# xfause/OpenGL_Ray_Tracing

Hardware: AMD Instinct MI355X
Metric: Mrays/sec + ms/frame (1 spp, 1080p) at 1/2/4/8 MI355X; CPU-ref spp-matched PSNR (higher is better)
Workload: dtype f32; 1 GPU; c2: OpenglRayTracing bunny scene (5k tris), 1080p, 1 spp/frame, Lambert; resolution=1920x1080, spp_per_frame=1, integrator=lambert, max_bounce=2, triangles=5004, bvh_nodes=2826, bvh_builder=sah, env=peppermint, traversal_tree=runtime (checked against uploaded), frame_kernel=path regeneration, frames_in_flight=2, hw_queues=4, frames_per_launch=12, parallelism=screen-tile x1

## Files before the change

opengl_ray_tracing_amd/csrc/pt_device.h:

```cpp
#pragma once
#include <hip/hip_runtime.h>
#include <stdint.h>

#include "pt_fmath.h"
#include "pt_kernels.h"

#define PT_PI 3.1415926f
#define PT_INF 2147483647.0f

namespace pt {

struct V3 {
  float x, y, z;
};
__device__ __forceinline__ V3 v3(float x, float y, float z) { return V3{x, y, z}; }
__device__ __forceinline__ V3 operator+(V3 a, V3 b) { return v3(a.x + b.x, a.y + b.y, a.z + b.z); }
__device__ __forceinline__ V3 operator-(V3 a, V3 b) { return v3(a.x - b.x, a.y - b.y, a.z - b.z); }
__device__ __forceinline__ V3 operator*(V3 a, V3 b) { return v3(a.x * b.x, a.y * b.y, a.z * b.z); }
__device__ __forceinline__ V3 operator*(V3 a, float s) { return v3(a.x * s, a.y * s, a.z * s); }
__device__ __forceinline__ V3 operator/(V3 a, float s) { return v3(a.x / s, a.y / s, a.z / s); }
__device__ __forceinline__ V3 operator-(V3 a) { return v3(-a.x, -a.y, -a.z); }
__device__ __forceinline__ float dot(V3 a, V3 b) { return (a.x * b.x + a.y * b.y) + a.z * b.z; }
__device__ __forceinline__ V3 cross(V3 a, V3 b) {
  return v3(a.y * b.z - b.y * a.z, a.z * b.x - b.z * a.x, a.x * b.y - b.x * a.y);
// ... 206 lines not shown
  b = b + 0.5f;
  u = a;
  w = 1.0f - b;
}
__device__ __noinline__ int sphTexelExact(int W, int H, V3 v) {
  float u, w;
  toSpherical(v, u, w);
  return texIndex(W, H, u, w);
}
__device__ __forceinline__ int sphTexel(int W, int H, V3 v) {
  float a = ptm_atan2f_fast(v.z, v.x), b = ptm_asinf_fast(v.y);
  a = a / (2.0f * PT_PI);
  b = b / PT_PI;
  a = a + 0.5f;
  b = b + 0.5f;
  const float fx = a * (float)W, fy = (1.0f - b) * (float)H;
  if (fabsf(fx - rintf(fx)) > 4e-7f * (float)W && fabsf(fy - rintf(fy)) > 4e-7f * (float)H) {
    const int x = (int)fminf(fmaxf(floorf(fx), 0.0f), (float)(W - 1));
    const int y = (int)fminf(fmaxf(floorf(fy), 0.0f), (float)(H - 1));
    return y * W + x;
  }
  return sphTexelExact(W, H, v);
}
__device__ __forceinline__ V3 sampleHdr(const Env& e, V3 v) {
  if (!e.hdr) return v3(0, 0, 0);
  float4 c = envTexelK(e, sphTexel(e.w, e.h, normalize(v)));
  return v3(fminf(c.x, 10.0f), fminf(c.y, 10.0f), fminf(c.z, 10.0f));
}
__device__ __forceinline__ V3 hdrColor(const Env& e, V3 L) {
  if (!e.hdr) return v3(0, 0, 0);
  float u, w;
  toSpherical(normalize(L), u, w);
  float4 c = envTexel(e, u, w);
  return v3(c.x, c.y, c.z);
}
__device__ __forceinline__ float2 hdrCacheTexel(const Env& e, float xi1, float xi2) {
  if (!e.cache) return make_float2(0.0f, 0.0f);
  if (e.cacheRow) {
    int col, row;
    texXY(e.w, e.h, xi1, xi2, col, row);
    const uint32_t r = e.cacheRow[row];
    const uint32_t y = e.cacheY[(size_t)(r >> 16) * e.w + (col & ((PT_DIAG_ENV_SMALL & 2) ? 1023 : -1))];
    return decodeCache4((r & 0xffffu) | y << 16, e.w, e.h);
  }
  const int k = texIndex(e.w, e.h, xi1, xi2) & ((PT_DIAG_ENV_SMALL & 2) ? 1023 : -1);
  if (e.nt) return e.cache4 ? decodeCache4(ldStream(e.cache4 + k), e.w, e.h) : ldStream(e.cache + k);
  return e.cache4 ? decodeCache4(e.cache4[k], e.w, e.h) : e.cache[k];
}
__device__ __forceinline__ float hdrTheta(float y) { return PT_PI * ((1.0f - y) - 0.5f); }
__device__ __forceinline__ float hdrPhi(float x) { return 2.0f * PT_PI * (x - 0.5f); }
// ... 288 lines not shown
```

opengl_ray_tracing_amd/csrc/pt_display.hip:

```cpp
#include <hip/hip_runtime.h>

#include <stdint.h>

#include "pt_device.h"
#include "pt_frame.h"
#include "pt_kernels.h"

namespace pt {

__global__ void tonemapKernel(const float4* accum, float* rgb, int n, float limit, float gamma) {
  int i = blockIdx.x * blockDim.x + threadIdx.x;
  if (i >= n) return;
  const V3 c = tonemapPixel(accum[i], limit, gamma);
  rgb[3 * i] = c.x;
  rgb[3 * i + 1] = c.y;
  rgb[3 * i + 2] = c.z;
}
hipError_t launchTonemap(const float4* accum, float* rgb, int n, float limit, float gamma, hipStream_t s) {
  hipLaunchKernelGGL(tonemapKernel, dim3((n + 255) / 256), dim3(256), 0, s, accum, rgb, n, limit, gamma);
  return hipGetLastError();
}
__device__ __forceinline__ uint32_t unorm8(float x) {
  const float c = fminf(fmaxf(x, 0.0f), 1.0f);
  return (uint32_t)__builtin_fmaf(c, 255.0f, 0.5f);
// ... 138 lines not shown
  if (!src) return;
  PackParams p = d.base;
  p.share.rank = rank;
  p.count = d.count[rank];
  long k = (long)blockIdx.x * blockDim.x + threadIdx.x;
  if (k >= p.count) return;
  int px, py;
  if (!pixelOfSlot(p.share, k, px, py)) return;
  const float* in = src + PACK_STATS_F * k;
  const size_t i = (size_t)py * p.share.width + px;
  stStream(accum + i, make_float4(in[0], in[1], in[2], 1.0f));
  stStream(moments + i, make_float2(in[3], in[4]));
}
hipError_t launchUnpackRanksStats(const RanksUnpack& d, int world, float4* accum, float2* moments, hipStream_t s) {
  if (!accum || !moments) return hipErrorInvalidValue;
  long most = 0;
  for (int k = 1; k < world; k++) most = d.count[k] > most ? d.count[k] : most;
  if (world < 2 || most <= 0) return hipSuccess;
  hipLaunchKernelGGL(unpackRanksStatsKernel, dim3((unsigned)((most + 255) / 256), (unsigned)(world - 1)), dim3(256), 0,
                     s, d, accum, moments);
  return hipGetLastError();
}

template <bool MOMENTS, bool ADAPTIVE = false>
__device__ __forceinline__ void mixFrames(const PackParams& p, float4* accum, float2* moments, const float* col,
                                          size_t colStride, int nFrames, uint32_t frameCounter,
                                          const uint32_t* retiredAt = nullptr) {
  long k = (long)blockIdx.x * blockDim.x + threadIdx.x;
  if (k >= p.count) return;
  int px, py;
  if (!pixelOfSlot(p.share, k, px, py)) return;
  if (ADAPTIVE && retiredAt[(size_t)(py >> 3) * ((p.share.width + 7) >> 3) + (px >> 3)] != 0u) return;
  const size_t i = (size_t)py * p.share.width + px;
  float4 a = ldStream(accum + i);
  float2 m = make_float2(0.0f, 0.0f);
  if (MOMENTS) m = ldStream(moments + i);
  for (int f = 0; f < nFrames; f++) {
    const float3 c = ldCol(col + ((size_t)f * colStride + k) * COL_F);
    const float w = 1.0f / (float)(frameCounter + (uint32_t)f + 1u);
    a = make_float4(mixf(a.x, c.x, w), mixf(a.y, c.y, w), mixf(a.z, c.z, w), 1.0f);
    if (MOMENTS) {
      const float l = (0.3f * c.x + 0.6f * c.y) + 0.1f * c.z;
      m = make_float2(mixf(m.x, l, w), mixf(m.y, l * l, w));
    }
  }
  stStream(accum + i, a);
  if (MOMENTS) stStream(moments + i, m);
}
__global__ void mixKernel(PackParams p, float4* accum, const float* col, size_t colStride, int nFrames,
                          uint32_t frameCounter) {
  mixFrames<false>(p, accum, nullptr, col, colStride, nFrames, frameCounter);
}
__global__ void mixMomentsKernel(PackParams p, float4* accum, float2* moments, const float* col, size_t colStride,
                                 int nFrames, uint32_t frameCounter) {
  mixFrames<true>(p, accum, moments, col, colStride, nFrames, frameCounter);
}
__global__ void mixAdaptiveKernel(PackParams p, float4* accum, float2* moments, const float* col, size_t colStride,
                                  int nFrames, uint32_t frameCounter, const uint32_t* retiredAt) {
  mixFrames<true, true>(p, accum, moments, col, colStride, nFrames, frameCounter, retiredAt);
}
hipError_t launchMix(const PackParams& p, float4* accum, const float* col, size_t colStride, int nFrames,
                     uint32_t frameCounter, hipStream_t s) {
  if (p.count <= 0 || nFrames <= 0) return hipSuccess;
  hipLaunchKernelGGL(mixKernel, dim3((unsigned)((p.count + 255) / 256)), dim3(256), 0, s, p, accum, col, colStride,
                     nFrames, frameCounter);
  return hipGetLastError();
}
hipError_t launchMixMoments(const PackParams& p, float4* accum, float2* moments, const float* col, size_t colStride,
                            int nFrames, uint32_t frameCounter, hipStream_t s) {
  if (p.count <= 0 || nFrames <= 0) return hipSuccess;
  hipLaunchKernelGGL(mixMomentsKernel, dim3((unsigned)((p.count + 255) / 256)), dim3(256), 0, s, p, accum, moments, col,
                     colStride, nFrames, frameCounter);
  return hipGetLastError();
}
hipError_t launchMixAdaptive(const PackParams& p, float4* accum, float2* moments, const float* col, size_t colStride,
                             int nFrames, uint32_t frameCounter, const uint32_t* retiredAt, hipStream_t s) {
  if (!retiredAt) return hipErrorInvalidValue;
  if (p.count <= 0 || nFrames <= 0) return hipSuccess;
  hipLaunchKernelGGL(mixAdaptiveKernel, dim3((unsigned)((p.count + 255) / 256)), dim3(256), 0, s, p, accum, moments,
                     col, colStride, nFrames, frameCounter, retiredAt);
  return hipGetLastError();
}

}
```

opengl_ray_tracing_amd/csrc/pt_kernels.h:

```cpp
#pragma once
#include <hip/hip_runtime.h>
#include <stdint.h>

namespace pt {

#ifndef PT_BLOCK
#define PT_BLOCK 256
#endif
constexpr int BLOCK = PT_BLOCK;
#ifndef PT_LDS_STACK
#define PT_LDS_STACK 32
#endif
#ifndef PT_MIN_WAVES_LAMBERT
#define PT_MIN_WAVES_LAMBERT 3
#endif
#ifndef PT_COST_EMA
#define PT_COST_EMA 2
#endif
#ifndef PT_WIDE_SCENE_MB
#define PT_WIDE_SCENE_MB 48
#endif
constexpr int WIDE_WAVES = 3;
#ifndef PT_WIDE_REGEN_WAVES
#define PT_WIDE_REGEN_WAVES 4
// ... 234 lines not shown
  const void* src[DISPLAY_MAX_WORLD];
  long count[DISPLAY_MAX_WORLD];
};

#ifndef PT_BIN_CAP
#define PT_BIN_CAP 32
#endif
#ifndef PT_PASS_BIN_CAP
#define PT_PASS_BIN_CAP 64
#endif
#ifndef PT_BINS
#define PT_BINS 1
#endif
struct PrimaryBins {
  int4* rect = nullptr;
  int* triCount = nullptr;
  int* triOffset = nullptr;
  int* tileCount = nullptr;
  int* binStart = nullptr;
  int* binTris = nullptr;
  float4* binGeo = nullptr;
  float4* binBox = nullptr;
  void* tmp = nullptr;
  size_t rectCap = 0, triCountCap = 0, triOffsetCap = 0, tileCountCap = 0, binStartCap = 0, binTrisCap = 0,
         binGeoCap = 0, binBoxCap = 0, tmpBytes = 0;
  int tilesX = 0, tilesY = 0, entries = 0;
};
hipError_t buildPrimaryBins(const float eye[3], const float cam[16], int width, int height, const float4* geo,
                            const float4* leafBox, int nTri, PrimaryBins& b, hipStream_t s);
void freePrimaryBins(PrimaryBins& b);

struct BuildNode {
  float4 lo;
  float4 hi;
  float4 clo;
  float4 chi;
};
struct AccelBuild {
  float4* bvh = nullptr;
  float4* pairs = nullptr;
  int* order = nullptr;
  BuildNode* nodes = nullptr;
  int rootRef = REF_NONE, nDev = 0, depth = 0, nNodes = 0;
};
hipError_t buildAccelDevice(const float4* geo, int nTri, int leafSize, float inflate, float inflateRelAbs,
                            AccelBuild& out, hipStream_t s);
void freeAccelBuild(AccelBuild& a);
hipError_t collapseWide4Device(const BuildNode* nodes, int nNodes, int leafSize, float inflate, float inflateRelAbs,
                               float4** out, int* rootRef, int* nDev, int* depth, hipStream_t s);

struct RefitTables {
  int2* topo = nullptr;
// ... 34 lines not shown
  const float* mats;
  int stride;
  int nTri;
  float4* hitRec;
  float4* table;
};
int materialSlots(int nTri);
hipError_t materialScanBytes(int nTri, size_t* bytes);
hipError_t launchMaterials(const MaterialParams& p, const MaterialTables& t, hipEvent_t* ev, hipStream_t s);

hipError_t launchHdrCache(const float* hdr, int w, int h, float4* cache, float* scratch, hipStream_t s);
hipError_t launchEnvCompact(const float4* hdr, const float2* cache, int w, int h, uint2* hdr8, uint32_t* cache4,
                            int* bad, hipStream_t s);
hipError_t launchEnvPack(float4* hdr, const float4* cache, float2* samp, int n, hipStream_t s);
hipError_t launchEnvTrig(float2* trig, int w, int h, hipStream_t s);
hipError_t launchEnvLight(const Env& e, uint2* light, hipStream_t s);
hipError_t launchRender(const RenderParams& p, int integrator, int grid, hipStream_t s, bool cull, bool count,
                        bool wide = false);
constexpr int REORDER_MAX = 4096;
hipError_t launchReorder(int* cost, int* costMax, int* splitLg, int* ema, int* order, int perQueue, int orderCap,
                         int numItems, int group, int numWaves, int splitPct, hipStream_t s);
hipError_t renderBlocksPerCU(int integrator, bool cull, bool count, bool wide, int* nb);
constexpr int PRIM_MISS = -1, PRIM_RETRACE = -2, PRIM_TILE = -3;
hipError_t launchPrimary(const RenderParams& p, hipStream_t s);
hipError_t launchLiveList(const RenderParams& p, hipStream_t s);
struct RegenVariant {
  const void* fn = nullptr;
  int waves = 0;
  int block = BLOCK;
  bool lists = true;
  int top4 = 0;
};
struct RegenShape {
  bool wide = false;
  bool fullTree = false;
  bool small = false;
  RegenVariant v;
  int blocksPerCU = 0;
  size_t dynLds = 0;
};
hipError_t regenShape(int integrator, bool cull, bool wide, int f4nDev, bool smallScene, RegenShape* out);
hipError_t launchRegen(const RenderParams& p, int integrator, int grid, hipStream_t s, bool cull, const RegenShape& r);
bool regenTakesLists(int integrator, const RegenShape& r);
int regenLdsStack();
int regenTop4(const RegenShape& r, int integrator);
hipError_t launchQuery(const QueryParams& p, int grid, hipStream_t s, bool occluded, bool cull);
struct GuideParams {
// ... 65 lines not shown
  float sigmaZ, normalCos, maxHistory;
  float frames;
};
constexpr int TEMPORAL_TILE = 16;
hipError_t launchTemporal(const TemporalParams& p, hipStream_t s);
hipError_t launchBasic(const BasicParams& p, hipStream_t s);
hipError_t launchBasicWiden(const float4* accum, double* image, long n, hipStream_t s);
hipError_t launchBasicNarrow(const double* image, float4* accum, long n, hipStream_t s);
hipError_t launchTonemap(const float4* accum, float* rgb, int n, float limit, float gamma, hipStream_t s);
constexpr int PACK_F = 3;
hipError_t launchPack(const PackParams& p, const float4* accum, float* packed, hipStream_t s);
hipError_t launchFmath(int fn, const float* x, const float* y, int n, float* out, hipStream_t s);
hipError_t launchSphTexel(int W, int H, const float* dirs, int n, int* texel, int* texelExact, hipStream_t s);
hipError_t launchDisplayPack(const PackParams& p, const float4* accum, float limit, float gamma, uint8_t* packed,
                             hipStream_t s);
hipError_t launchDisplayOwn(const PackParams& p, const float4* accum, float limit, float gamma, uchar4* image,
                            hipStream_t s);
hipError_t launchDisplayUnpack(const RanksUnpack& d, int world, uchar4* image, hipStream_t s);
hipError_t launchUnpackRanks(const RanksUnpack& d, int world, float4* accum, hipStream_t s);
hipError_t launchUnpack(const PackParams& p, float4* accum, const float* packed, hipStream_t s);
constexpr int PACK_STATS_F = 5;
hipError_t launchPackStats(const PackParams& p, const float4* accum, const float2* moments, float* packed, hipStream_t s);
hipError_t launchUnpackRanksStats(const RanksUnpack& d, int world, float4* accum, float2* moments, hipStream_t s);
hipError_t launchMix(const PackParams& p, float4* accum, const float* col, size_t colStride, int nFrames,
                     uint32_t frameCounter, hipStream_t s);
hipError_t launchMixMoments(const PackParams& p, float4* accum, float2* moments, const float* col, size_t colStride,
                            int nFrames, uint32_t frameCounter, hipStream_t s);
hipError_t launchMixAdaptive(const PackParams& p, float4* accum, float2* moments, const float* col, size_t colStride,
                             int nFrames, uint32_t frameCounter, const uint32_t* retiredAt, hipStream_t s);
struct TileErrorParams {
  Share share;
  int shardTiles;
  int waveTiles;
  int tilesX;
  const float4* accum;
  const float2* moments;
  float* err2;
  uint32_t* retiredAt;
  float kf;
  float limit;
  float thr2;
  uint32_t frames;
  int minFrames;
};
hipError_t launchTileError(const TileErrorParams& p, hipStream_t s);

}
```

opengl_ray_tracing_amd/csrc/pt_primary.hip:

```cpp
#include <hip/hip_runtime.h>
#include <hipcub/hipcub.hpp>
#include <stdint.h>

#include "pt_frame.h"
#include "pt_kernels.h"
#include "pt_trace.h"

namespace pt {

struct BinCam {
  double eye[3];
  double R[9];
  int width, height, tilesX, tilesY;
};

constexpr double kNearZ = -2.5e-4;
constexpr double kMarginPx = 2.0;

__device__ __forceinline__ void toCam(const BinCam& c, const float4 v, double q[3]) {
  const double r0 = (double)v.x - c.eye[0], r1 = (double)v.y - c.eye[1], r2 = (double)v.z - c.eye[2];
  for (int a = 0; a < 3; a++) q[a] = c.R[3 * a] * r0 + c.R[3 * a + 1] * r1 + c.R[3 * a + 2] * r2;
}

__global__ void binRectKernel(BinCam c, const float4* geo, int nTri, int4* rect, int* count) {
// ... 135 lines not shown
  if ((e = hipMemcpyAsync(&entries, b.triOffset + nTri, sizeof(int), hipMemcpyDeviceToHost, s)) != hipSuccess) return e;
  if ((e = hipStreamSynchronize(s)) != hipSuccess) return e;
  if ((e = grow(b.binTris, b.binTrisCap, (size_t)std::max(entries, 1))) != hipSuccess) return e;
  if ((e = hipMemsetAsync(b.tileCount, 0, ((size_t)nTiles + 1) * sizeof(int), s)) != hipSuccess) return e;
  if (entries > 0)
    hipLaunchKernelGGL(binCountKernel, dim3((entries + B - 1) / B), dim3(B), 0, s, b.triOffset, b.rect, nTri, c.tilesX,
                       entries, b.tileCount);
  if ((e = scanInts(b.tileCount, b.binStart, nTiles, b.tmp, b.tmpBytes, s)) != hipSuccess) return e;
  if ((e = hipMemsetAsync(b.tileCount, 0, ((size_t)nTiles + 1) * sizeof(int), s)) != hipSuccess) return e;
  if (entries > 0)
    hipLaunchKernelGGL(binFillKernel, dim3((entries + B - 1) / B), dim3(B), 0, s, b.triOffset, b.rect, nTri, c.tilesX,
                       entries, b.binStart, b.tileCount, b.binTris);
  if ((e = grow(b.binGeo, b.binGeoCap, 4 * (size_t)std::max(entries, 1))) != hipSuccess) return e;
  if ((e = grow(b.binBox, b.binBoxCap, 2 * (size_t)std::max(entries, 1))) != hipSuccess) return e;
  if (entries > 0 && leafBox)
    hipLaunchKernelGGL(binGatherKernel, dim3((entries + B - 1) / B), dim3(B), 0, s, b.binTris, entries, geo, leafBox,
                       b.binGeo, b.binBox);
  b.tilesX = c.tilesX;
  b.tilesY = c.tilesY;
  b.entries = entries;
  return hipGetLastError();
}

void freePrimaryBins(PrimaryBins& b) {
  for (void* p : {(void*)b.rect, (void*)b.triCount, (void*)b.triOffset, (void*)b.tileCount, (void*)b.binStart,
                  (void*)b.binTris, (void*)b.binGeo, (void*)b.binBox, b.tmp})
    if (p) (void)hipFree(p);
  b = PrimaryBins{};
}

__global__ __launch_bounds__(64) void primaryKernel(RenderParams p) {
  __shared__ float4 s_tri[PT_PASS_BIN_CAP * 4];
  __shared__ float4 s_box[PT_PASS_BIN_CAP * 2];
  __shared__ int s_idx[PT_PASS_BIN_CAP];
  const int fr = (int)(blockIdx.x % (unsigned)p.nFrames);
  const int w = (int)(blockIdx.x / (unsigned)p.nFrames);
  const int lane = threadIdx.x;
  if (p.zeroQueue && blockIdx.x == 0)
    for (int q = lane; q < NUM_QUEUES; q += 64) p.queue[q * CTL_LINE_INTS] = 0;
  const int2 o = tileOrigin(shareOf(p), w, p.shardTiles);
  const int px = o.x + (lane & 7);
  const int py = o.y + (lane >> 3);
  const bool valid = px < p.width && py < p.height;
  const int tx = o.x >> 3, ty = o.y >> 3;
  int b0 = 0, b1 = 0;
  uint32_t gone = 0u;
  if (tx < p.binTilesX && ty < p.binTilesY) {
    b0 = p.binStart[ty * p.binTilesX + tx];
    b1 = p.binStart[ty * p.binTilesX + tx + 1];
    if (p.retiredAt) gone = p.retiredAt[ty * p.binTilesX + tx];
  }
  if (gone != 0u) {
    if (lane == 0) p.primMask[(size_t)fr * p.numItems + w] = 0ull;
    return;
  }
  const int n = b1 - b0;
  int2* out = p.primHit + ((size_t)fr * p.numItems + w) * 64;
  unsigned long long* mask = p.primMask + (size_t)fr * p.numItems + w;
  const FrameRef fp = frameRef(p, fr);
// ... 16 lines not shown
  const V3 eye = v3(p.eye[0], p.eye[1], p.eye[2]);
  float tbest;
  int best;
  bool tie;
  closestInBin(n, valid, eye, dir, [&](int k) { return s_tri + 4 * k; }, tbest, best, tie);
  uint32_t rays = 0;
  int res = PRIM_MISS;
  if (valid) {
    res = best >= 0 ? s_idx[best] : PRIM_MISS;
    if (tie || (res >= 0 && !refReachableBox(p.scene, s_box[2 * best], s_box[2 * best + 1], eye, dir, tbest))) {
      res = PRIM_RETRACE;
    } else {
      rays = 1;
      if (res == PRIM_MISS) storeSample(p, fp, px, py, sampleHdr(p.env, dir));
    }
  }
  const bool need = valid && res != PRIM_MISS;
  const unsigned long long m = __ballot(need);
  if (need) out[__popcll(m & ((1ull << lane) - 1ull))] = make_int2(res, __float_as_int(tbest));
  if (lane == 0) *mask = m;
  addRays(p.rayShards, rays);
}

hipError_t launchPrimary(const RenderParams& p, hipStream_t s) {
  if (!p.primHit || !p.primMask || !p.binStart || !p.binGeo || !p.binBox || p.numItems <= 0) return hipErrorInvalidValue;
  hipLaunchKernelGGL(primaryKernel, dim3((unsigned)p.numItems * (unsigned)p.nFrames), dim3(64), 0, s, p);
  return hipGetLastError();
}

constexpr int LIVE_BS = 1024;
__global__ __launch_bounds__(LIVE_BS) void liveListKernel(RenderParams p) {
  __shared__ int s_wave[LIVE_BS / 64];
  const int q = blockIdx.x, lane = threadIdx.x & 63, wv = threadIdx.x >> 6;
  const int nF = p.nFrames, total = p.perQueue * nF;
  uint4* seg = p.liveItems + (size_t)q * liveStride(p.perQueue, nF);
  uint4* out = seg + LIVE_HEAD;
  auto load = [&](int it, int& t, int& fr) -> unsigned long long {
    const int k = it / nF;
    fr = it - k * nF;
    t = q * p.perQueue + k;
    return it < total && t < p.numItems ? p.primMask[(size_t)fr * p.numItems + t] : 0ull;
  };
  int base = 0;
  int t, fr;
  unsigned long long m = load((int)threadIdx.x, t, fr);
  for (int it0 = 0; it0 < total; it0 += LIVE_BS) {
    int tn, frn;
    const unsigned long long mn = load(it0 + LIVE_BS + (int)threadIdx.x, tn, frn);
    const unsigned long long b = __ballot(m != 0);
// ... 27 lines not shown
```

opengl_ray_tracing_amd/csrc/pt_runtime.cpp:

```cpp
#include <hip/hip_runtime.h>

#include <algorithm>
#include <cstdio>
#include <cstdlib>
#include <cstring>
#include <string>
#include <vector>

#include "pt_abi.h"
#include "pt_kernels.h"
#include "pt_plan.h"
#include "pt_runtime.h"

using namespace pt;

#ifndef PT_DIRECT_SOLO
#define PT_DIRECT_SOLO 1
#endif
static_assert(PT_PIPE >= 1 && PT_PIPE <= PIPE, "PT_PIPE: 1..MAX_SLOTS");
static_assert(PIPE * NUM_QUEUES * CTL_LINE_INTS * 4 <= (int)CTL_STATS, "queue counters of every slot fit the control block");

template <class T, class Bytes, class Wait>
static int frameBuffer(pt_ctx* ctx, T** bufs, int* caps, int n, int idx, int frames, int cap, Bytes bytes, Wait wait) {
  auto alloc = [&](int k) -> int {
// ... 335 lines not shown
  p.stats = reinterpret_cast<unsigned long long*>(ctx->d_ctl + CTL_STATS);
  p.rayShards = reinterpret_cast<unsigned long long*>(ctx->d_ctl + CTL_RAYS);
  return p;
}

static int tileOrderLists(pt_ctx* ctx, bool ordered, int slot, int** cost, int** order) {
  const int orderCap = 4 * ctx->perQueue + 64;
  const size_t orderInts = (size_t)NUM_QUEUES * orderCap + NUM_QUEUES;
  ctx->orderCap = orderCap;
  if (!ordered) return PT_OK;
  if (!ctx->d_cost) {
    const size_t n = (size_t)PIPE * ctx->numItems * 4;
    CK(hipMalloc(&ctx->d_cost, n * sizeof(int)));
    CK(hipMemset(ctx->d_cost, 0, n * sizeof(int)));
    CK(hipMalloc(&ctx->d_order, (size_t)PIPE * orderInts * sizeof(int)));
    for (int k = 0; k < PIPE; k++) ctx->orderValid[k] = false;
  }
  *cost = ctx->d_cost + (size_t)slot * 4 * ctx->numItems;
  *order = ctx->d_order + (size_t)slot * orderInts;
  return PT_OK;
}

static int bindBins(pt_ctx* ctx, const FramePlan& pl, const FrameSlot& at, const RegenShape& rs, int nF,
                    const float eye[3], const float cameraRotate[16], RenderParams* p) {
  const pt_config& c = ctx->cfg;
  hipStream_t S = at.S;
  if (!ctx->binsValid || ctx->binVersion != ctx->sceneVersion || std::memcmp(ctx->binEye, eye, sizeof(ctx->binEye)) ||
      std::memcmp(ctx->binCam, cameraRotate, sizeof(ctx->binCam))) {
    if (pl.piped) {
      if (int e = waitOthers(ctx, at)) return e;
    }
    ctx->binsValid = false;
    CK(buildPrimaryBins(eye, cameraRotate, c.width, c.height, ctx->d_geo, ctx->d_leafBox, ctx->nTri, ctx->bins, S));
    std::memcpy(ctx->binEye, eye, sizeof(ctx->binEye));
    std::memcpy(ctx->binCam, cameraRotate, sizeof(ctx->binCam));
    ctx->binVersion = ctx->sceneVersion;
    ctx->binsValid = true;
    if (pl.piped) {
      CK(hipEventRecord(ctx->binsBuilt, S));
      ctx->binGen++;
      ctx->binGenSeen[at.slot] = ctx->binGen;
    }
  }
  if (pl.piped && ctx->binGenSeen[at.slot] != ctx->binGen) {
    CK(hipStreamWaitEvent(S, ctx->binsBuilt, 0));
    ctx->binGenSeen[at.slot] = ctx->binGen;
  }
  p->binStart = ctx->bins.binStart;
  p->binTris = ctx->bins.binTris;
  p->binGeo = ctx->bins.binGeo;
  p->binBox = ctx->bins.binBox;
  p->binTilesX = ctx->bins.tilesX;
  p->binTilesY = ctx->bins.tilesY;
  if (!pl.pass) return PT_OK;
  const int n = pl.piped ? at.D : 0, cap = std::max(nF, pl.piped ? ctx->batchCap : 1);
  auto waitSlot = [&]() { return hipStreamSynchronize(S); };
  const size_t primBytes = p->colStride * sizeof(int2) + (size_t)ctx->numItems * sizeof(unsigned long long);
  if (int rc = frameBuffer(ctx, ctx->d_prim, ctx->primCap, n, at.slot, nF, cap,
                           [&](int f) { return (size_t)f * primBytes; }, waitSlot))
    return rc;
  p->primHit = ctx->d_prim[at.slot];
  p->primMask = reinterpret_cast<unsigned long long*>(ctx->d_prim[at.slot] + (size_t)ctx->primCap[at.slot] * p->colStride);
  if (pl.regen && regenTakesLists(c.integrator, rs)) {
    if (int rc = frameBuffer(ctx, ctx->d_live, ctx->liveCap, n, at.slot, nF, cap,
                             [&](int f) { return (size_t)NUM_QUEUES * liveStride(ctx->perQueue, f) * sizeof(uint4); },
                             waitSlot))
      return rc;
    p->liveItems = p->primHit ? ctx->d_live[at.slot] : nullptr;
  }
  return PT_OK;
}

static int enqueueFrame(pt_ctx* ctx, const FramePlan& pl, const FrameSlot& at, const LaunchShape& g, RenderParams& p,
                        int* cost, int* order, int split) {
  const pt_config& c = ctx->cfg;
  hipStream_t S = at.S;
  hipEvent_t evb, eve;
  int erc = launchEvents(ctx, &evb, &eve);
  if (erc) return erc;
#if PT_WAVE_TRACE
  const size_t nTrace = (size_t)g.grid * (g.bs / 64) * WAVE_TRACE_WORDS;
  unsigned long long* dTrace = nullptr;
  {
    CK(hipMalloc(&dTrace, nTrace * sizeof(unsigned long long)));
    CK(hipMemsetAsync(dTrace, 0, nTrace * sizeof(unsigned long long), S));
  }
  p.waveTrace = dTrace;
#endif
  p.zeroQueue = p.primHit != nullptr;
  if (!p.primHit) CK(hipMemsetAsync(p.queue, 0, (size_t)NUM_QUEUES * CTL_LINE_INTS * sizeof(int), S));
  CK(hipEventRecord(evb, S));
  if (p.primHit) CK(launchPrimary(p, S));
  if (p.liveItems) CK(launchLiveList(p, S));
  if (pl.regen) CK(launchRegen(p, c.integrator, g.grid, S, pl.cull, g.rs));
  else CK(launchRender(p, c.integrator, g.grid, S, pl.cull, pl.count, pl.wide));
#if PT_WAVE_TRACE
  if (dTrace) {
    std::vector<unsigned long long> tr(nTrace);
    CK(hipMemcpyAsync(tr.data(), dTrace, nTrace * sizeof(unsigned long long), hipMemcpyDeviceToHost, S));
    CK(hipStreamSynchronize(S));
    (void)hipFree(dTrace);
    if (const char* fn = std::getenv("PT_WAVE_TRACE_FILE")) {
      if (FILE* f = std::fopen(fn, "ab")) {
        std::fwrite(tr.data(), sizeof(unsigned long long), nTrace, f);
        std::fclose(f);
      }
    }
  }
#endif
  if (pl.ordered) {
    CK(launchReorder(cost, cost + ctx->numItems, cost + 2 * (size_t)ctx->numItems, cost + 3 * (size_t)ctx->numItems,
                     order, ctx->perQueue, ctx->orderCap, ctx->numItems, std::max(1, PT_TILE_GROUP),
                     g.grid * (BLOCK / 64), split, S));
    ctx->orderValid[at.slot] = true;
    ctx->orderSplit[at.slot] = split > 0;
  }
  CK(hipEventRecord(eve, S));
  return PT_OK;
}

static int enqueueMix(pt_ctx* ctx, const FrameSlot& at, int nF, bool direct, uint32_t frameCounter) {
  const pt_config& c = ctx->cfg;
  const int slot = at.slot, colIdx = at.colIdx;
  const size_t shareN = (size_t)ctx->numItems * 64;
  CK(hipEventRecord(ctx->kernelDone[slot], at.S));
  ctx->slotBusy[slot] = true;
  if (at.S != ctx->slotStream[slot])
    CK(hipStreamWaitEvent(ctx->slotStream[slot], ctx->kernelDone[slot], 0));
  if (at.S != ctx->stream) CK(hipStreamWaitEvent(ctx->stream, ctx->kernelDone[slot], 0));
  if (ctx->mixPending && ctx->lastMixStream != ctx->stream)
    CK(hipStreamWaitEvent(ctx->stream, ctx->mixDone[ctx->lastCol], 0));
  ctx->lastMixStream = ctx->stream;
  if (ctx->d_mom) {
    if (ctx->d_retiredAt) {
      if (int rc = joinAdaptive(ctx)) return rc;
      CK(launchMixAdaptive(packParams(ctx, c.tile_rank, c.tile_world), ctx->d_accum, ctx->d_mom, ctx->d_col[colIdx],
                           shareN, nF, frameCounter, ctx->d_retiredAt, ctx->stream));
    } else {
      CK(launchMixMoments(packParams(ctx, c.tile_rank, c.tile_world), ctx->d_accum, ctx->d_mom, ctx->d_col[colIdx],
                          shareN, nF, frameCounter, ctx->stream));
    }
    ctx->momFrames = frameCounter == 0 ? (uint32_t)nF : (frameCounter == ctx->momFrames ? ctx->momFrames + (uint32_t)nF : 0u);
  } else if (!direct)
    CK(launchMix(packParams(ctx, c.tile_rank, c.tile_world), ctx->d_accum, ctx->d_col[colIdx], shareN, nF,
                 frameCounter, ctx->stream));
  CK(hipEventRecord(ctx->mixDone[colIdx], ctx->stream));
  ctx->lastSlot = slot;
  ctx->lastCol = colIdx;
  ctx->mixPending = true;
  ctx->frameNo++;
  return PT_OK;
}

static int renderOne(pt_ctx* ctx, const float eye[3], const float cameraRotate[16], uint32_t frameCounter,
                     int want = 1, int* done = nullptr) {
  if (!ctx) return PT_E_INVALID;
  if (done) *done = 1;
  CK(hipSetDevice(ctx->cfg.device_id));
  const pt_config& c = ctx->cfg;
  if (c.integrator == PT_BASIC_CPU_COMPAT) return renderBasic(ctx, frameCounter);
  if (!ctx->d_bvh || !eye || !cameraRotate) return fail(ctx, ctx->d_bvh ? PT_E_INVALID : PT_E_NOSCENE, "no scene");
  FrameSlot at;
  const bool piped = pipedFrames(ctx);
  if (piped) {
    if (int e = ensureSlots(ctx, ctx->pipeDepth)) return e;
    at.D = ctx->pipeDepth;
    at.slot = (int)(ctx->frameNo % (unsigned)at.D);
    at.nCol = 2 * at.D + 1;
// ... 24 lines not shown
  p.packets = PT_PACKETS && (useFast ? ctx->fDepth : ctx->depth) + 1 <= PKT_DEPTH;
  const bool probing = pl.ordered && PT_SPLIT_AUTO && (ctx->treeDecided < 0 || ctx->splitDecided < 0);
  const int nF = piped && !probing ? std::max(1, std::min(want, ctx->batchCap)) : 1;
  if (done) *done = nF;
  p.nFrames = nF;
  const bool direct = piped && at.solo && nF == 1 && !pl.regen && PT_DIRECT_SOLO && !ctx->d_mom;
  if (direct && ctx->mixPending && ctx->lastMixStream != S) CK(hipStreamWaitEvent(S, ctx->mixDone[ctx->lastCol], 0));
  if (piped) {
    if (int rc = frameBuffer(ctx, ctx->d_col, ctx->colCap, at.nCol, at.colIdx, nF, std::max(nF, ctx->batchCap),
                             [&](int f) { return (size_t)f * p.colStride * COL_F * sizeof(float); },
                             [&]() { return hipEventSynchronize(ctx->mixDone[at.colIdx]); }))
      return rc;
  }
  p.col = piped && !direct ? ctx->d_col[at.colIdx] : nullptr;
  if (ctx->d_retiredAt) {
    if (frameCounter == 0)
      if (int rc = clearAdaptive(ctx)) return rc;
    if (ctx->adaptGenSeen[at.slot] != ctx->adaptGen) {
      CK(hipStreamWaitEvent(S, ctx->adaptDone, 0));
      ctx->adaptGenSeen[at.slot] = ctx->adaptGen;
    }
    p.retiredAt = ctx->d_retiredAt;
  }
  if (pl.bins)
    if (int rc = bindBins(ctx, pl, at, g.rs, nF, eye, cameraRotate, &p)) return rc;
  const bool splitThis = nF == 1;
  p.tileOrder = pl.ordered && ctx->orderValid[at.slot] && !(!splitThis && ctx->orderSplit[at.slot]) ? order : nullptr;
  p.orderCap = ctx->orderCap;
  p.tileCost = cost;
  p.tileCostMax = pl.ordered ? cost + ctx->numItems : nullptr;
  if (piped && probing) {
    if (int e = waitOthers(ctx, at)) return e;
  }
  if (int rc = enqueueFrame(ctx, pl, at, g, p, cost, order, splitThis ? splitPct : 0)) return rc;
  if (piped)
    if (int rc = enqueueMix(ctx, at, nF, direct, frameCounter)) return rc;
  commitLaunch(ctx, nF);
  return PT_OK;
}

int joinPipe(pt_ctx* ctx) {
  if (!ctx->mixPending) return PT_OK;
  CK(hipSetDevice(ctx->cfg.device_id));
  CK(hipStreamWaitEvent(ctx->stream, ctx->mixDone[ctx->lastCol], 0));
  return PT_OK;
}

int syncStreams(pt_ctx* ctx) {
  CK(hipSetDevice(ctx->cfg.device_id));
  for (int k = 0; k < PIPE; k++) {
    if (ctx->slotStream[k]) CK(hipStreamSynchronize(ctx->slotStream[k]));
    ctx->slotBusy[k] = false;
  }
  CK(hipStreamSynchronize(ctx->stream));
  ctx->mixPending = false;
  return PT_OK;
}

int pt_render_frames_async(pt_ctx* ctx, const float eye[3], const float cameraRotate[16], uint32_t frameCounter,
// ... 29 lines not shown
```

opengl_ray_tracing_amd/csrc/pt_runtime.h:

```cpp
#pragma once
#include <hip/hip_runtime.h>

#include <string>
#include <vector>

#include "pt_abi.h"
#include "pt_envupdate.h"
#include "pt_frame.h"
#include "pt_kernels.h"
#include "pt_rccl.h"

using namespace pt;

static constexpr int EV_RING = 64;
#ifndef PT_PIPE
#define PT_PIPE 8
#endif
static constexpr int PIPE = MAX_SLOTS;
static constexpr int COLS = 2 * MAX_SLOTS + 1;

struct pt_ctx {
  pt_config cfg{};
  std::string err;
  hipStream_t own = nullptr, stream = nullptr;
// ... 65 lines not shown
  int lastWaves = 0;
  int probeFrame = 0;
  PrimaryBins bins;
  bool binsValid = false;
  float binEye[3] = {}, binCam[16] = {};
  unsigned sceneVersion = 0, binVersion = 0;
  bool pipe = false;
  int pipeDepth = PT_PIPE;
  int pipeDepthBase = PT_PIPE;
  bool pipeDepthFixed = false;
  int batchCap = 1;
  int colCap[COLS] = {};
  int primCap[PIPE] = {};
  int liveCap[PIPE] = {};
  int regenWide = -1;
  bool solo = true;
  hipStream_t slotStream[PIPE] = {};
  hipEvent_t kernelDone[PIPE] = {};
  bool slotBusy[PIPE] = {};
  hipEvent_t mixDone[COLS] = {};
  hipStream_t lastMixStream = nullptr;
  hipEvent_t binsBuilt = nullptr;
  unsigned binGen = 0, binGenSeen[MAX_SLOTS] = {};
  float* d_col[COLS] = {};
  int2* d_prim[PIPE] = {};
  uint4* d_live[PIPE] = {};
  int lastSlot = -1;
  int lastCol = -1;
  bool mixPending = false;
  unsigned long long frameNo = 0;
  int probeN[4] = {0, 0, 0, 0};
  double probeMs[4] = {0.0, 0.0, 0.0, 0.0};
  long long probeLast[4] = {-1, -1, -1, -1};
  int probeGen = 0;
  int treeDecided = -1, splitDecided = -1;
  unsigned policyKey = 0, probedKey = ~0u;
  int orderCap = 0;
  bool orderValid[PIPE] = {};
  bool orderSplit[PIPE] = {};
  size_t ovfInts = 0;
  int shardSize = 32, shardsX = 0, shardsY = 0, numItems = 0, perQueue = 0;
  float* d_rgb = nullptr;
  int* d_queryOvf = nullptr;
  size_t queryOvfInts = 0;
  hipEvent_t queryDone = nullptr;
  hipStream_t queryStream = nullptr;
// ... 115 lines not shown
```

Baseline: 21100 Mrays/s.

## Skip primary pass for empty bin tiles and shade sky-only pixels in mix

Builds a compacted list of screen tiles whose primary bins contain triangles, and launches the primary-visibility kernel only over those tiles. Pixels in empty tiles are resolved in the mix kernel by regenerating the camera ray and sampling the HDR environment directly, batching texel loads in chunks of four and counting the rays via sharded atomics. The goal is to avoid tracing and writing per-frame colour for background-only tiles, which make up much of a bunny scene. The cost is a host sync after each pass-list build, a primMask memset whenever the bins are rebuilt, and more complexity and register pressure in the mix kernel.

```diff
diff --git a/opengl_ray_tracing_amd/csrc/pt_device.h b/opengl_ray_tracing_amd/csrc/pt_device.h
--- a/opengl_ray_tracing_amd/csrc/pt_device.h
+++ b/opengl_ray_tracing_amd/csrc/pt_device.h
@@ -252,10 +252,38 @@
   }
   return sphTexelExact(W, H, v);
 }
+__device__ __forceinline__ int sampleHdrTexel(const Env& e, V3 v) { return sphTexel(e.w, e.h, normalize(v)); }
+__device__ __forceinline__ V3 skyOfTexel(float4 c) { return v3(fminf(c.x, 10.0f), fminf(c.y, 10.0f), fminf(c.z, 10.0f)); }
 __device__ __forceinline__ V3 sampleHdr(const Env& e, V3 v) {
   if (!e.hdr) return v3(0, 0, 0);
-  float4 c = envTexelK(e, sphTexel(e.w, e.h, normalize(v)));
-  return v3(fminf(c.x, 10.0f), fminf(c.y, 10.0f), fminf(c.z, 10.0f));
+  return skyOfTexel(envTexelK(e, sampleHdrTexel(e, v)));
+}
+template <int N>
+__device__ __forceinline__ void sampleHdrAt(const Env& e, const int (&k)[N], V3 (&out)[N]) {
+  const int mask = (PT_DIAG_ENV_SMALL & 1) ? 1023 : -1;
+  if (e.hdr8) {
+    uint2 t[N];
+    if (e.nt) {
+#pragma unroll
+      for (int j = 0; j < N; j++) t[j] = ldStream(e.hdr8 + (k[j] & mask));
+    } else {
+#pragma unroll
+      for (int j = 0; j < N; j++) t[j] = e.hdr8[k[j] & mask];
+    }
+#pragma unroll
+    for (int j = 0; j < N; j++) out[j] = skyOfTexel(decodeHdr8(t[j]));
+  } else {
+    float4 t[N];
+    if (e.nt) {
+#pragma unroll
+      for (int j = 0; j < N; j++) t[j] = ldStream(e.hdr + (k[j] & mask));
+    } else {
+#pragma unroll
+      for (int j = 0; j < N; j++) t[j] = e.hdr[k[j] & mask];
+    }
+#pragma unroll
+    for (int j = 0; j < N; j++) out[j] = skyOfTexel(t[j]);
+  }
 }
 __device__ __forceinline__ V3 hdrColor(const Env& e, V3 L) {
   if (!e.hdr) return v3(0, 0, 0);
diff --git a/opengl_ray_tracing_amd/csrc/pt_display.hip b/opengl_ray_tracing_amd/csrc/pt_display.hip
--- a/opengl_ray_tracing_amd/csrc/pt_display.hip
+++ b/opengl_ray_tracing_amd/csrc/pt_display.hip
@@ -184,64 +184,106 @@
   return hipGetLastError();
 }
 
-template <bool MOMENTS, bool ADAPTIVE = false>
+constexpr int SKY_CHUNK = 4;
+template <bool MOMENTS, bool ADAPTIVE, bool SKY>
 __device__ __forceinline__ void mixFrames(const PackParams& p, float4* accum, float2* moments, const float* col,
-                                          size_t colStride, int nFrames, uint32_t frameCounter,
-                                          const uint32_t* retiredAt = nullptr) {
-  long k = (long)blockIdx.x * blockDim.x + threadIdx.x;
-  if (k >= p.count) return;
-  int px, py;
-  if (!pixelOfSlot(p.share, k, px, py)) return;
-  if (ADAPTIVE && retiredAt[(size_t)(py >> 3) * ((p.share.width + 7) >> 3) + (px >> 3)] != 0u) return;
+                                          size_t colStride, int nFrames, uint32_t frameCounter, const SkyTiles& sky,
+                                          const uint32_t* retiredAt) {
+  long k = (long)blockIdx.x * blockDim.x + threadIdx.x;
+  int px = 0, py = 0;
+  bool on = k < p.count && pixelOfSlot(p.share, k, px, py);
+  if (ADAPTIVE && on && retiredAt[(size_t)(py >> 3) * ((p.share.width + 7) >> 3) + (px >> 3)] != 0u) on = false;
+  bool own = false;
+  if (SKY) {
+    if (on) {
+      const int t = (py >> 3) * sky.binTilesX + (px >> 3);
+      own = sky.binStart[t + 1] == sky.binStart[t];
+    }
+    const unsigned long long b = __ballot(own);
+    if ((threadIdx.x & 63) == 0 && b)
+      atomicAdd(sky.rayShards + (blockIdx.x & (RAY_SHARDS - 1)) * RAY_SHARD_STRIDE,
+                (unsigned long long)__popcll(b) * (unsigned long long)nFrames);
+  }
+  if (!on) return;
   const size_t i = (size_t)py * p.share.width + px;
   float4 a = ldStream(accum + i);
   float2 m = make_float2(0.0f, 0.0f);
   if (MOMENTS) m = ldStream(moments + i);
-  for (int f = 0; f < nFrames; f++) {
-    const float3 c = ldCol(col + ((size_t)f * colStride + k) * COL_F);
+  auto mix = [&](int f, float cx, float cy, float cz) {
     const float w = 1.0f / (float)(frameCounter + (uint32_t)f + 1u);
-    a = make_float4(mixf(a.x, c.x, w), mixf(a.y, c.y, w), mixf(a.z, c.z, w), 1.0f);
+    a = make_float4(mixf(a.x, cx, w), mixf(a.y, cy, w), mixf(a.z, cz, w), 1.0f);
     if (MOMENTS) {
-      const float l = (0.3f * c.x + 0.6f * c.y) + 0.1f * c.z;
+      const float l = (0.3f * cx + 0.6f * cy) + 0.1f * cz;
       m = make_float2(mixf(m.x, l, w), mixf(m.y, l * l, w));
+    }
+  };
+  if (!SKY || !own) {
+    for (int f = 0; f < nFrames; f++) {
+      const float3 c = ldCol(col + ((size_t)f * colStride + k) * COL_F);
+      mix(f, c.x, c.y, c.z);
+    }
+  } else if (!sky.env.hdr) {
+    for (int f = 0; f < nFrames; f++) mix(f, 0.0f, 0.0f, 0.0f);
+  } else {
+    for (int f0 = 0; f0 < nFrames; f0 += SKY_CHUNK) {
+      int tex[SKY_CHUNK];
+#pragma unroll
+      for (int j = 0; j < SKY_CHUNK; j++) {
+        const int f = min(f0 + j, nFrames - 1);
+        uint32_t seed;
+        const V3 dir = cameraRay(sky.cam, p.share.width, p.share.height, sky.sampleIndex + (uint32_t)f * sky.sampleStride,
+                                 px, py, seed);
+        tex[j] = sampleHdrTexel(sky.env, dir);
+      }
+      V3 c[SKY_CHUNK];
+      sampleHdrAt(sky.env, tex, c);
+#pragma unroll
+      for (int j = 0; j < SKY_CHUNK; j++)
+        if (f0 + j < nFrames) mix(f0 + j, c[j].x, c[j].y, c[j].z);
     }
   }
   stStream(accum + i, a);
   if (MOMENTS) stStream(moments + i, m);
 }
+template <bool SKY>
 __global__ void mixKernel(PackParams p, float4* accum, const float* col, size_t colStride, int nFrames,
-                          uint32_t frameCounter) {
-  mixFrames<false>(p, accum, nullptr, col, colStride, nFrames, frameCounter);
-}
+                          uint32_t frameCounter, SkyTiles sky) {
+  mixFrames<false, false, SKY>(p, accum, nullptr, col, colStride, nFrames, frameCounter, sky, nullptr);
+}
+template <bool SKY>
 __global__ void mixMomentsKernel(PackParams p, float4* accum, float2* moments, const float* col, size_t colStride,
-                                 int nFrames, uint32_t frameCounter) {
-  mixFrames<true>(p, accum, moments, col, colStride, nFrames, frameCounter);
-}
+                                 int nFrames, uint32_t frameCounter, SkyTiles sky) {
+  mixFrames<true, false, SKY>(p, accum, moments, col, colStride, nFrames, frameCounter, sky, nullptr);
+}
+template <bool SKY>
 __global__ void mixAdaptiveKernel(PackParams p, float4* accum, float2* moments, const float* col, size_t colStride,
-                                  int nFrames, uint32_t frameCounter, const uint32_t* retiredAt) {
-  mixFrames<true, true>(p, accum, moments, col, colStride, nFrames, frameCounter, retiredAt);
+                                  int nFrames, uint32_t frameCounter, const uint32_t* retiredAt, SkyTiles sky) {
+  mixFrames<true, true, SKY>(p, accum, moments, col, colStride, nFrames, frameCounter, sky, retiredAt);
 }
 hipError_t launchMix(const PackParams& p, float4* accum, const float* col, size_t colStride, int nFrames,
-                     uint32_t frameCounter, hipStream_t s) {
+                     uint32_t frameCounter, const SkyTiles& sky, hipStream_t s) {
+  if (sky.binStart && !sky.rayShards) return hipErrorInvalidValue;
   if (p.count <= 0 || nFrames <= 0) return hipSuccess;
-  hipLaunchKernelGGL(mixKernel, dim3((unsigned)((p.count + 255) / 256)), dim3(256), 0, s, p, accum, col, colStride,
-                     nFrames, frameCounter);
+  hipLaunchKernelGGL(sky.binStart ? mixKernel<true> : mixKernel<false>, dim3((unsigned)((p.count + 255) / 256)), dim3(256), 0, s, p, accum, col, colStride,
+                     nFrames, frameCounter, sky);
   return hipGetLastError();
 }
 hipError_t launchMixMoments(const PackParams& p, float4* accum, float2* moments, const float* col, size_t colStride,
-                            int nFrames, uint32_t frameCounter, hipStream_t s) {
+                            int nFrames, uint32_t frameCounter, const SkyTiles& sky, hipStream_t s) {
+  if (sky.binStart && !sky.rayShards) return hipErrorInvalidValue;
   if (p.count <= 0 || nFrames <= 0) return hipSuccess;
-  hipLaunchKernelGGL(mixMomentsKernel, dim3((unsigned)((p.count + 255) / 256)), dim3(256), 0, s, p, accum, moments, col,
-                     colStride, nFrames, frameCounter);
+  hipLaunchKernelGGL(sky.binStart ? mixMomentsKernel<true> : mixMomentsKernel<false>, dim3((unsigned)((p.count + 255) / 256)), dim3(256), 0, s, p, accum, moments, col,
+                     colStride, nFrames, frameCounter, sky);
   return hipGetLastError();
 }
 hipError_t launchMixAdaptive(const PackParams& p, float4* accum, float2* moments, const float* col, size_t colStride,
-                             int nFrames, uint32_t frameCounter, const uint32_t* retiredAt, hipStream_t s) {
-  if (!retiredAt) return hipErrorInvalidValue;
+                             int nFrames, uint32_t frameCounter, const uint32_t* retiredAt, const SkyTiles& sky,
+                             hipStream_t s) {
+  if (!retiredAt || (sky.binStart && !sky.rayShards)) return hipErrorInvalidValue;
   if (p.count <= 0 || nFrames <= 0) return hipSuccess;
-  hipLaunchKernelGGL(mixAdaptiveKernel, dim3((unsigned)((p.count + 255) / 256)), dim3(256), 0, s, p, accum, moments,
-                     col, colStride, nFrames, frameCounter, retiredAt);
-  return hipGetLastError();
-}
-
-}
+  hipLaunchKernelGGL(sky.binStart ? mixAdaptiveKernel<true> : mixAdaptiveKernel<false>, dim3((unsigned)((p.count + 255) / 256)), dim3(256), 0, s, p, accum, moments,
+                     col, colStride, nFrames, frameCounter, retiredAt, sky);
+  return hipGetLastError();
+}
+
+}
diff --git a/opengl_ray_tracing_amd/csrc/pt_kernels.h b/opengl_ray_tracing_amd/csrc/pt_kernels.h
--- a/opengl_ray_tracing_amd/csrc/pt_kernels.h
+++ b/opengl_ray_tracing_amd/csrc/pt_kernels.h
@@ -280,12 +280,15 @@
   float4* binGeo = nullptr;
   float4* binBox = nullptr;
   void* tmp = nullptr;
+  int* passList = nullptr;
   size_t rectCap = 0, triCountCap = 0, triOffsetCap = 0, tileCountCap = 0, binStartCap = 0, binTrisCap = 0,
-         binGeoCap = 0, binBoxCap = 0, tmpBytes = 0;
+         binGeoCap = 0, binBoxCap = 0, tmpBytes = 0, passListCap = 0;
   int tilesX = 0, tilesY = 0, entries = 0;
+  int passCount = 0;
 };
 hipError_t buildPrimaryBins(const float eye[3], const float cam[16], int width, int height, const float4* geo,
                             const float4* leafBox, int nTri, PrimaryBins& b, hipStream_t s);
+hipError_t buildPassList(const Share& share, PrimaryBins& b, hipStream_t s);
 void freePrimaryBins(PrimaryBins& b);
 
 struct BuildNode {
@@ -366,7 +369,7 @@
                          int numItems, int group, int numWaves, int splitPct, hipStream_t s);
 hipError_t renderBlocksPerCU(int integrator, bool cull, bool count, bool wide, int* nb);
 constexpr int PRIM_MISS = -1, PRIM_RETRACE = -2, PRIM_TILE = -3;
-hipError_t launchPrimary(const RenderParams& p, hipStream_t s);
+hipError_t launchPrimary(const RenderParams& p, const int* passList, int passCount, hipStream_t s);
 hipError_t launchLiveList(const RenderParams& p, hipStream_t s);
 struct RegenVariant {
   const void* fn = nullptr;
@@ -478,12 +481,22 @@
 constexpr int PACK_STATS_F = 5;
 hipError_t launchPackStats(const PackParams& p, const float4* accum, const float2* moments, float* packed, hipStream_t s);
 hipError_t launchUnpackRanksStats(const RanksUnpack& d, int world, float4* accum, float2* moments, hipStream_t s);
+struct SkyTiles {
+  const int* binStart;
+  int binTilesX;
+  uint32_t sampleIndex;
+  uint32_t sampleStride;
+  float cam[16];
+  Env env;
+  unsigned long long* rayShards;
+};
 hipError_t launchMix(const PackParams& p, float4* accum, const float* col, size_t colStride, int nFrames,
-                     uint32_t frameCounter, hipStream_t s);
+                     uint32_t frameCounter, const SkyTiles& sky, hipStream_t s);
 hipError_t launchMixMoments(const PackParams& p, float4* accum, float2* moments, const float* col, size_t colStride,
-                            int nFrames, uint32_t frameCounter, hipStream_t s);
+                            int nFrames, uint32_t frameCounter, const SkyTiles& sky, hipStream_t s);
 hipError_t launchMixAdaptive(const PackParams& p, float4* accum, float2* moments, const float* col, size_t colStride,
-                             int nFrames, uint32_t frameCounter, const uint32_t* retiredAt, hipStream_t s);
+                             int nFrames, uint32_t frameCounter, const uint32_t* retiredAt, const SkyTiles& sky,
+                             hipStream_t s);
 struct TileErrorParams {
   Share share;
   int shardTiles;
diff --git a/opengl_ray_tracing_amd/csrc/pt_primary.hip b/opengl_ray_tracing_amd/csrc/pt_primary.hip
--- a/opengl_ray_tracing_amd/csrc/pt_primary.hip
+++ b/opengl_ray_tracing_amd/csrc/pt_primary.hip
@@ -181,19 +181,73 @@
   return hipGetLastError();
 }
 
+constexpr int PASS_BS = 1024;
+__global__ __launch_bounds__(PASS_BS) void passListKernel(Share share, int per, int numItems, const int* binStart,
+                                                          int tilesX, int tilesY, int* list) {
+  __shared__ int s_wave[PASS_BS / 64];
+  const int lane = threadIdx.x & 63, wv = threadIdx.x >> 6;
+  int base = 0;
+  for (int w0 = 0; w0 < numItems; w0 += PASS_BS) {
+    const int w = w0 + (int)threadIdx.x;
+    bool in = false;
+    if (w < numItems) {
+      const int2 o = tileOrigin(share, w, per);
+      const int tx = o.x >> 3, ty = o.y >> 3;
+      if (tx < tilesX && ty < tilesY) in = binStart[ty * tilesX + tx + 1] > binStart[ty * tilesX + tx];
+    }
+    const unsigned long long b = __ballot(in);
+    if (lane == 0) s_wave[wv] = __popcll(b);
+    __syncthreads();
+    int before = 0, all = 0;
+    for (int k = 0; k < PASS_BS / 64; k++) {
+      const int c = s_wave[k];
+      before += k < wv ? c : 0;
+      all += c;
+    }
+    if (in) list[base + before + __popcll(b & ((1ull << lane) - 1ull))] = w;
+    base += all;
+    __syncthreads();
+  }
+  if (threadIdx.x == 0) list[numItems] = base;
+}
+
+hipError_t buildPassList(const Share& share, PrimaryBins& b, hipStream_t s) {
+  const int numItems = waveTiles(share);
+  b.passCount = 0;
+  if (numItems <= 0) return hipSuccess;
+  if (!b.binStart) return hipErrorInvalidValue;
+  hipError_t e;
+  if ((size_t)numItems + 1 > b.passListCap) {
+    if (b.passList) (void)hipFree(b.passList);
+    b.passList = nullptr;
+    b.passListCap = 0;
+    if ((e = hipMalloc(&b.passList, ((size_t)numItems + 1) * sizeof(int))) != hipSuccess) return e;
+    b.passListCap = (size_t)numItems + 1;
+  }
+  hipLaunchKernelGGL(passListKernel, dim3(1), dim3(PASS_BS), 0, s, share, shardTiles(share), numItems, b.binStart,
+                     b.tilesX, b.tilesY, b.passList);
+  if ((e = hipGetLastError()) != hipSuccess) return e;
+  int count = 0;
+  if ((e = hipMemcpyAsync(&count, b.passList + numItems, sizeof(int), hipMemcpyDeviceToHost, s)) != hipSuccess) return e;
+  if ((e = hipStreamSynchronize(s)) != hipSuccess) return e;
+  b.passCount = count;
+  return hipSuccess;
+}
+
 void freePrimaryBins(PrimaryBins& b) {
   for (void* p : {(void*)b.rect, (void*)b.triCount, (void*)b.triOffset, (void*)b.tileCount, (void*)b.binStart,
-                  (void*)b.binTris, (void*)b.binGeo, (void*)b.binBox, b.tmp})
+                  (void*)b.binTris, (void*)b.binGeo, (void*)b.binBox, (void*)b.passList, b.tmp})
     if (p) (void)hipFree(p);
   b = PrimaryBins{};
 }
 
-__global__ __launch_bounds__(64) void primaryKernel(RenderParams p) {
+__global__ __launch_bounds__(64) void primaryKernel(RenderParams p, const int* passList) {
   __shared__ float4 s_tri[PT_PASS_BIN_CAP * 4];
   __shared__ float4 s_box[PT_PASS_BIN_CAP * 2];
   __shared__ int s_idx[PT_PASS_BIN_CAP];
   const int fr = (int)(blockIdx.x % (unsigned)p.nFrames);
-  const int w = (int)(blockIdx.x / (unsigned)p.nFrames);
+  const int item = (int)(blockIdx.x / (unsigned)p.nFrames);
+  const int w = passList ? passList[item] : item;
   const int lane = threadIdx.x;
   if (p.zeroQueue && blockIdx.x == 0)
     for (int q = lane; q < NUM_QUEUES; q += 64) p.queue[q * CTL_LINE_INTS] = 0;
@@ -256,9 +310,11 @@
   addRays(p.rayShards, rays);
 }
 
-hipError_t launchPrimary(const RenderParams& p, hipStream_t s) {
+hipError_t launchPrimary(const RenderParams& p, const int* passList, int passCount, hipStream_t s) {
   if (!p.primHit || !p.primMask || !p.binStart || !p.binGeo || !p.binBox || p.numItems <= 0) return hipErrorInvalidValue;
-  hipLaunchKernelGGL(primaryKernel, dim3((unsigned)p.numItems * (unsigned)p.nFrames), dim3(64), 0, s, p);
+  if (passList && (passCount <= 0 || passCount > p.numItems)) return hipErrorInvalidValue;
+  const unsigned tiles = passList ? (unsigned)passCount : (unsigned)p.numItems;
+  hipLaunchKernelGGL(primaryKernel, dim3(tiles * (unsigned)p.nFrames), dim3(64), 0, s, p, passList);
   return hipGetLastError();
 }
 
diff --git a/opengl_ray_tracing_amd/csrc/pt_runtime.cpp b/opengl_ray_tracing_amd/csrc/pt_runtime.cpp
--- a/opengl_ray_tracing_amd/csrc/pt_runtime.cpp
+++ b/opengl_ray_tracing_amd/csrc/pt_runtime.cpp
@@ -381,16 +381,19 @@
 }
 
 static int bindBins(pt_ctx* ctx, const FramePlan& pl, const FrameSlot& at, const RegenShape& rs, int nF,
-                    const float eye[3], const float cameraRotate[16], RenderParams* p) {
+                    const float eye[3], const float cameraRotate[16], RenderParams* p, SkyTiles* sky) {
   const pt_config& c = ctx->cfg;
   hipStream_t S = at.S;
   if (!ctx->binsValid || ctx->binVersion != ctx->sceneVersion || std::memcmp(ctx->binEye, eye, sizeof(ctx->binEye)) ||
       std::memcmp(ctx->binCam, cameraRotate, sizeof(ctx->binCam))) {
     if (pl.piped) {
       if (int e = waitOthers(ctx, at)) return e;
+      if (ctx->mixPending && S != ctx->lastMixStream) CK(hipStreamWaitEvent(S, ctx->mixDone[ctx->lastCol], 0));
     }
     ctx->binsValid = false;
     CK(buildPrimaryBins(eye, cameraRotate, c.width, c.height, ctx->d_geo, ctx->d_leafBox, ctx->nTri, ctx->bins, S));
+    CK(buildPassList(shareOf(ctx, c.tile_rank, c.tile_world), ctx->bins, S));
+    ctx->binBuilds++;
     std::memcpy(ctx->binEye, eye, sizeof(ctx->binEye));
     std::memcpy(ctx->binCam, cameraRotate, sizeof(ctx->binCam));
     ctx->binVersion = ctx->sceneVersion;
@@ -420,6 +423,22 @@
     return rc;
   p->primHit = ctx->d_prim[at.slot];
   p->primMask = reinterpret_cast<unsigned long long*>(ctx->d_prim[at.slot] + (size_t)ctx->primCap[at.slot] * p->colStride);
+  if (p->col && p->primHit && !pl.wideScene) {
+    sky->binStart = ctx->bins.binStart;
+    sky->binTilesX = ctx->bins.tilesX;
+    sky->sampleIndex = p->sampleIndex;
+    sky->sampleStride = p->sampleStride;
+    std::memcpy(sky->cam, cameraRotate, sizeof(sky->cam));
+    sky->env = p->env;
+    sky->rayShards = p->rayShards;
+    const int k = at.slot;
+    if (ctx->maskBuild[k] != ctx->binBuilds || ctx->maskBuf[k] != ctx->d_prim[k] || ctx->maskCap[k] != ctx->primCap[k]) {
+      CK(hipMemsetAsync(p->primMask, 0, (size_t)ctx->primCap[k] * ctx->numItems * sizeof(unsigned long long), S));
+      ctx->maskBuild[k] = ctx->binBuilds;
+      ctx->maskBuf[k] = ctx->d_prim[k];
+      ctx->maskCap[k] = ctx->primCap[k];
+    }
+  }
   if (pl.regen && regenTakesLists(c.integrator, rs)) {
     if (int rc = frameBuffer(ctx, ctx->d_live, ctx->liveCap, n, at.slot, nF, cap,
                              [&](int f) { return (size_t)NUM_QUEUES * liveStride(ctx->perQueue, f) * sizeof(uint4); },
@@ -431,7 +450,7 @@
 }
 
 static int enqueueFrame(pt_ctx* ctx, const FramePlan& pl, const FrameSlot& at, const LaunchShape& g, RenderParams& p,
-                        int* cost, int* order, int split) {
+                        const SkyTiles& sky, int* cost, int* order, int split) {
   const pt_config& c = ctx->cfg;
   hipStream_t S = at.S;
   hipEvent_t evb, eve;
@@ -446,10 +465,12 @@
   }
   p.waveTrace = dTrace;
 #endif
-  p.zeroQueue = p.primHit != nullptr;
-  if (!p.primHit) CK(hipMemsetAsync(p.queue, 0, (size_t)NUM_QUEUES * CTL_LINE_INTS * sizeof(int), S));
+  const int* passList = sky.binStart ? ctx->bins.passList : nullptr;
+  const bool passRuns = p.primHit && !(passList && ctx->bins.passCount == 0);
+  p.zeroQueue = passRuns;
+  if (!passRuns) CK(hipMemsetAsync(p.queue, 0, (size_t)NUM_QUEUES * CTL_LINE_INTS * sizeof(int), S));
   CK(hipEventRecord(evb, S));
-  if (p.primHit) CK(launchPrimary(p, S));
+  if (passRuns) CK(launchPrimary(p, passList, ctx->bins.passCount, S));
   if (p.liveItems) CK(launchLiveList(p, S));
   if (pl.regen) CK(launchRegen(p, c.integrator, g.grid, S, pl.cull, g.rs));
   else CK(launchRender(p, c.integrator, g.grid, S, pl.cull, pl.count, pl.wide));
@@ -478,7 +499,7 @@
   return PT_OK;
 }
 
-static int enqueueMix(pt_ctx* ctx, const FrameSlot& at, int nF, bool direct, uint32_t frameCounter) {
+static int enqueueMix(pt_ctx* ctx, const FrameSlot& at, int nF, bool direct, uint32_t frameCounter, const SkyTiles& sky) {
   const pt_config& c = ctx->cfg;
   const int slot = at.slot, colIdx = at.colIdx;
   const size_t shareN = (size_t)ctx->numItems * 64;
@@ -494,15 +515,15 @@
     if (ctx->d_retiredAt) {
       if (int rc = joinAdaptive(ctx)) return rc;
       CK(launchMixAdaptive(packParams(ctx, c.tile_rank, c.tile_world), ctx->d_accum, ctx->d_mom, ctx->d_col[colIdx],
-                           shareN, nF, frameCounter, ctx->d_retiredAt, ctx->stream));
+                           shareN, nF, frameCounter, ctx->d_retiredAt, sky, ctx->stream));
     } else {
       CK(launchMixMoments(packParams(ctx, c.tile_rank, c.tile_world), ctx->d_accum, ctx->d_mom, ctx->d_col[colIdx],
-                          shareN, nF, frameCounter, ctx->stream));
+                          shareN, nF, frameCounter, sky, ctx->stream));
     }
     ctx->momFrames = frameCounter == 0 ? (uint32_t)nF : (frameCounter == ctx->momFrames ? ctx->momFrames + (uint32_t)nF : 0u);
   } else if (!direct)
     CK(launchMix(packParams(ctx, c.tile_rank, c.tile_world), ctx->d_accum, ctx->d_col[colIdx], shareN, nF,
-                 frameCounter, ctx->stream));
+                 frameCounter, sky, ctx->stream));
   CK(hipEventRecord(ctx->mixDone[colIdx], ctx->stream));
   ctx->lastSlot = slot;
   ctx->lastCol = colIdx;
@@ -573,8 +594,10 @@
     }
     p.retiredAt = ctx->d_retiredAt;
   }
+  SkyTiles sky;
+  std::memset(&sky, 0, sizeof(sky));
   if (pl.bins)
-    if (int rc = bindBins(ctx, pl, at, g.rs, nF, eye, cameraRotate, &p)) return rc;
+    if (int rc = bindBins(ctx, pl, at, g.rs, nF, eye, cameraRotate, &p, &sky)) return rc;
   const bool splitThis = nF == 1;
   p.tileOrder = pl.ordered && ctx->orderValid[at.slot] && !(!splitThis && ctx->orderSplit[at.slot]) ? order : nullptr;
   p.orderCap = ctx->orderCap;
@@ -583,9 +606,9 @@
   if (piped && probing) {
     if (int e = waitOthers(ctx, at)) return e;
   }
-  if (int rc = enqueueFrame(ctx, pl, at, g, p, cost, order, splitThis ? splitPct : 0)) return rc;
+  if (int rc = enqueueFrame(ctx, pl, at, g, p, sky, cost, order, splitThis ? splitPct : 0)) return rc;
   if (piped)
-    if (int rc = enqueueMix(ctx, at, nF, direct, frameCounter)) return rc;
+    if (int rc = enqueueMix(ctx, at, nF, direct, frameCounter, sky)) return rc;
   commitLaunch(ctx, nF);
   return PT_OK;
 }
diff --git a/opengl_ray_tracing_amd/csrc/pt_runtime.h b/opengl_ray_tracing_amd/csrc/pt_runtime.h
--- a/opengl_ray_tracing_amd/csrc/pt_runtime.h
+++ b/opengl_ray_tracing_amd/csrc/pt_runtime.h
@@ -111,6 +111,9 @@
   hipStream_t lastMixStream = nullptr;
   hipEvent_t binsBuilt = nullptr;
   unsigned binGen = 0, binGenSeen[MAX_SLOTS] = {};
+  unsigned binBuilds = 0, maskBuild[PIPE] = {};
+  const void* maskBuf[PIPE] = {};
+  int maskCap[PIPE] = {};
   float* d_col[COLS] = {};
   int2* d_prim[PIPE] = {};
   uint4* d_live[PIPE] = {};
```

Result: faster. 22440 Mrays/s (median of 6 runs) (+6.4%).
